# smhassanerfani/nasa-niswan

Hardware: AMD Instinct MI355X
Metric: training samples/sec (90x144x20 grid, seq_len=12) (higher is better)
Workload: dtype bf16; 1 GPU; cfg1-20level; in_channels=62, out_channels=20, seq_len=12, batch_per_gpu=8, global_batch=8, parallelism=dp1, wave=4, overlap_allreduce=False

## Files before the change

nasa-niswan_amd/csrc/conv_igemm.hip:

```cpp
#include "nint_common.h"

enum { EPI_LSTM = 0, EPI_DGRAD = 1, EPI_DGRAD_PW = 2 };

#ifndef NINT_TINY_AUTO
#define NINT_TINY_AUTO(dtype) ((dtype) == NINT_F32)
#endif
#ifndef NINT_STENCIL_AUTO
#define NINT_STENCIL_AUTO(dtype) false
#endif

#ifndef NINT_BD
#define NINT_BD 3
#endif
constexpr int BD_WIDE = NINT_BD;
constexpr int BD_NARROW = 2;
#ifndef NINT_AG
#define NINT_AG 2
#endif
#ifndef NINT_ABUF
#define NINT_ABUF 2
#endif

#ifdef NINT_STAMP
#define NINT_STAMP_WGS 4096
// ... 11 lines not shown
extern "C" int nint_debug_read_hwid(unsigned* host, int n_wgs) {
  if (!host || n_wgs <= 0 || n_wgs > NINT_STAMP_WGS) return NINT_E_ARG;
  NINT_CHECK_HIP(hipDeviceSynchronize());
  NINT_CHECK_HIP(hipMemcpyFromSymbol(host, HIP_SYMBOL(g_hwid), (size_t)n_wgs * 2 * sizeof(unsigned)));
  return NINT_OK;
}
extern "C" int nint_debug_read_stamps(unsigned long long* host, int n_wgs) {
  if (!host || n_wgs <= 0 || n_wgs > NINT_STAMP_WGS) return NINT_E_ARG;
  NINT_CHECK_HIP(hipDeviceSynchronize());
  NINT_CHECK_HIP(hipMemcpyFromSymbol(host, HIP_SYMBOL(g_stamp), (size_t)n_wgs * 8 * sizeof(unsigned long long)));
  return NINT_OK;
}
#else
#define NINT_STAMP_AT(slot)
#endif

template <int DT> struct Pk4;
template <> struct Pk4<NINT_F32> {
  typedef f32x4_t T;
  static __device__ __forceinline__ T ld(const void* p, size_t i) { return *(const f32x4_t*)((const float*)p + i); }
  static __device__ __forceinline__ f32x4_t up(T v) { return v; }
  static __device__ __forceinline__ T zero() { return (f32x4_t){0.f, 0.f, 0.f, 0.f}; }
};
template <> struct Pk4<NINT_BF16> {
  typedef u32x2_t T;
  static __device__ __forceinline__ T ld(const void* p, size_t i) { return *(const u32x2_t*)((const uint16_t*)p + i); }
  static __device__ __forceinline__ f32x4_t up(T w) {
    return (f32x4_t){__builtin_bit_cast(float, w[0] << 16), __builtin_bit_cast(float, w[0] & 0xffff0000u),
                     __builtin_bit_cast(float, w[1] << 16), __builtin_bit_cast(float, w[1] & 0xffff0000u)};
  }
  static __device__ __forceinline__ T zero() { return (u32x2_t){0u, 0u}; }
};

constexpr int xchg_rounds(int EPI, int WK, int NTW, int MT) {
  return (WK == 4 && MT == 4 && NTW % 2 == 0) ? 2 : ((WK == 4 && MT == 8 && NTW == 4) ? 4 : 1);
}

template <int DT, int EPI, int WN, int WK, int NTW, int MT>
__device__ __forceinline__ void conv_igemm_body(const ConvArgs& a, char* smem, const int bx_, const int by_, const int nbx_) {
  static_assert(WN * WK == 4, "four waves per workgroup");
  constexpr int BD = MT >= 8 ? BD_WIDE : BD_NARROW;
  static_assert(EPI != EPI_LSTM || NTW % 4 == 0, "LSTM epilogue needs the 4 gate tiles in one wave");
  constexpr int NTH = 256;
  constexpr int NTWG = WN * NTW;
  constexpr int Q = MT / WK;
  static_assert(MT % WK == 0, "K-slice waves split the tile rows evenly");

  const int tid = threadIdx.x, lane = tid & 63;
  NINT_STAMP_AT(0)
  const int wave = __builtin_amdgcn_readfirstlane(tid >> 6);
  const int wn = wave % WN, wk = wave / WN;
  int tile;
  {
    const int nb = nbx_, b = bx_, q8 = nb / 8, r8 = nb % 8, x = b % 8, i = b / 8;
    tile = x * q8 + (x < r8 ? x : r8) + i;
  }
  const bool mg = MT >= 8 && tile >= a.n_full;
  int tx, ty, img;
  if (!mg) {
    tx = tile % a.tiles_x; tile /= a.tiles_x;
    ty = tile % a.tiles_full_y;
    img = tile / a.tiles_full_y;
  } else {
    tile -= a.n_full;
    tx = tile % a.tiles_x2;
    img = tile / a.tiles_x2;
    ty = a.tiles_full_y;
  }
  constexpr int RHM = MT >= 8 ? MT / 2 : MT;
  const int nt0 = a.nt_begin + by_ * NTWG + wn * NTW;
  const int y0 = ty * MT, x0 = mg ? tx * 32 : tx * 16;
  auto rdy = [&](int r) __attribute__((always_inline)) { return mg ? r % RHM : r; };
// ... 60 lines not shown
        const int r = (i + wk * Q) % MT;
        const int y = y0 + rdy(r), x = x0 + rdx(r) + (lane & 15);
        const size_t rowpix = ((size_t)img * a.H + y) * a.W;
#pragma unroll
        for (int j = 0; j < NTW; ++j) {
          const int n = (nt0 + j) * 16 + c4;
          old[i][j] = (f32x4_t){0.f, 0.f, 0.f, 0.f};
          if (rmw && n < a.C0p && y < a.H && x < a.W)
            old[i][j] = load_vec4<DT>(a.out0 + rowpix * a.C0p * Elem<DT>::ES, (unsigned)(x * a.C0p + n));
        }
      }
    }
  };
  if constexpr (EARLY) load_cprev();
  for (int c_begin = 0; c_begin < nchunks; c_begin += a.cpf) {
    const int c_cnt = min(a.cpf, nchunks - c_begin);
    if (c_begin > 0) __syncthreads();
    const int a_units = c_cnt * 4 * NHPp;
    for (int ub = wave * 64; ub < a_units; ub += 4 * 64) {
      const int u = ub + lane;
      const int cq = (int)__umulhi((unsigned)u, magic_nhpp);
      int hp = u - cq * NHPp;
      hp = hp < NHP ? hp : 0;
      const int q = cq & 3, cl = cq >> 2;
      const int hy = (int)__umulhi((unsigned)hp, magic_hwt);
      const int hx = hp - hy * HWt;
      const int c = c_begin + cl;
      const char* src = (c < a.nchunk0)
          ? base0 + ((long)hy * a.Wh + hx) * a.pix_stride0 + c * 64 + q * 16
          : base1 + ((long)hy * a.Wh + hx) * a.pix_stride1 + (c - a.nchunk0) * 64 + q * 16;
      __builtin_amdgcn_global_load_lds((const __attribute__((address_space(1))) void*)src,
                                       (__attribute__((address_space(3))) void*)(smem + (size_t)ub * 16), 16, 0, 0);
    }
    const int n0f = a.kx0 == k ? 0 : min(max(a.nchunk0 - c_begin, 0), c_cnt);
    const int steps_before = min(c_begin, a.nchunk0) * k * a.kx0 + max(c_begin - a.nchunk0, 0) * taps;
    bool synced = false;
    for (int seg = 0; seg < 2; ++seg) {
    const int cs_lo = seg == 0 ? 0 : n0f, cs_n = seg == 0 ? n0f : c_cnt - n0f;
    if (cs_n == 0) continue;
    const int kx = seg == 0 ? a.kx0 : k;
    const int xoff = kx == k ? 0 : p;
    const int tps = k * kx;
    const int nsteps = cs_n * tps;
    const int s_lo = (nsteps * wk) / WK, s_hi = (nsteps * (wk + 1)) / WK;
    int cl = s_lo / tps;
    int tap = s_lo - cl * tps;
    cl += cs_lo;
    int tyy = tap / kx;
    int txx = tap - tyy * kx;
    const char* Bs = Bwave + (size_t)(steps_before + (seg == 0 ? 0 : n0f * k * a.kx0) + s_lo) * bstep;
    u32x4_t bq[BD][NTW];
    int b_rem = s_hi - 1 - s_lo;
    const char* Bn = Bs;
#define NINT_B_ADVANCE() { const bool adv_ = b_rem > 0; b_rem -= adv_ ? 1 : 0; Bn += adv_ ? bstep : 0; }
    if (s_lo < s_hi) {
#pragma unroll
      for (int d = 0; d < BD; ++d) {
#pragma unroll
        for (int j = 0; j < NTW; ++j) bq[d][j] = *(const u32x4_t*)(Bn + blane + j * 1024);
        NINT_B_ADVANCE()
      }
    }
    if (!synced) {
      __syncthreads();
      synced = true;
      if (c_begin == 0) { NINT_STAMP_AT(1) }
// ... 90 lines not shown
    }
    }
  }

#undef NINT_B_ADVANCE
  NINT_STAMP_AT(2)
  if constexpr (WK > 1) {
    constexpr int FR = MT - Q;
    constexpr int XR = xchg_rounds(EPI, WK, NTW, MT), NTX = NTW / XR;
    __syncthreads();
#pragma unroll
    for (int xr = 0; xr < XR; ++xr) {
      if (xr > 0) __syncthreads();
      char* mine = smem + (size_t)((wn * WK + wk) * FR * NTX) * 1024 + lane * 16;
#pragma unroll
      for (int ii = Q; ii < MT; ++ii)
#pragma unroll
        for (int j = 0; j < NTX; ++j) *(f32x4_t*)(mine + ((ii - Q) * NTX + j) * 1024) = acc[ii][xr * NTX + j];
      __syncthreads();
#pragma unroll
      for (int d = 1; d < WK; ++d) {
        const int src = (wk + d) % WK;
        const int shift = ((wk - src + WK) % WK) * Q;
        const char* theirs = smem + (size_t)((wn * WK + src) * FR * NTX) * 1024 + lane * 16;
#pragma unroll
        for (int ii = 0; ii < Q; ++ii)
#pragma unroll
          for (int j = 0; j < NTX; ++j)
            acc[ii][xr * NTX + j] += *(const f32x4_t*)(theirs + ((ii + shift - Q) * NTX + j) * 1024);
      }
    }
  }

  if constexpr (!EARLY) load_cprev();
  load_old();
  const int px = lane & 15;
  const int c4 = 4 * (lane >> 4);
  const int x = x0 + px;
  if constexpr (EPI == EPI_LSTM) {
#pragma unroll
    for (int cb = 0; cb < NTW / 4; ++cb) {
      const int cblock = nt0 / 4 + cb;
      const int ch = cblock * 16 + c4;
      const int Gc = 4 * a.Ch16;
      const int odd = (lane >> 4) & 1, chb = (lane >> 5) * 8;
      const unsigned lo_c = (unsigned)(x * a.Chp + ch);
      const unsigned lo_h = (unsigned)((x + a.P) * a.Chp + ch);
      const unsigned lo_g = (unsigned)(x * Gc + cblock * 64) + (DT == NINT_BF16 ? (unsigned)(chb + (odd ? 32 : 0)) : (unsigned)c4);
#pragma unroll
      for (int i = 0; i < Q; ++i) {
        const int rt = (i + wk * Q) % MT;
        const int y = y0 + rdy(rt), xo = rdx(rt);
        const bool ok = y < a.H && x + xo < a.W;
        const size_t rowpix = ((size_t)img * a.H + y) * a.W + xo;
        const f32x4_t cp = cpv[i][cb];
        f32x4_t gi, gf, gg, go, cn, hn;
#pragma unroll
        for (int r = 0; r < 4; ++r) {
          gi[r] = sigmoidf_(acc[i][cb * 4 + 0][r]);
          gf[r] = sigmoidf_(acc[i][cb * 4 + 1][r]);
          gg[r] = tanhf_(acc[i][cb * 4 + 2][r]);
          go[r] = sigmoidf_(acc[i][cb * 4 + 3][r]);
          cn[r] = fmaf(cp[r], gf[r], gi[r] * gg[r]);
          hn[r] = go[r] * tanhf_(cn[r]);
        }
        if (ok) {
// ... 168 lines not shown
  int i = 0;                                                                                                    \
  _Pragma("unroll") for (int q = 1; q < NINT_MULTI_MAX; ++q) i += (q < m.n && (int)blockIdx.x >= m.begin[q]) ? 1 : 0; \
  const int b = blockIdx.x - m.begin[i];                                                                        \
  if (b >= m.nwg[i]) return;                                        \
  const int nbx = m.nbx[i], by = b / nbx, bx = b - by * nbx;                                                    \
  const ConvArgs& a = m.a[i];
#define NINT_MULTI_CASE(EPI_, WN_, WK_, NTW_) \
  case conv_variant(EPI_, WN_, WK_, NTW_, 4): conv_igemm_body<DT, EPI_, WN_, WK_, NTW_, 4>(a, smem, bx, by, nbx); break;
template <int DT>
__global__ __launch_bounds__(256, 3) void conv_lstm_multi_kernel(ConvMulti m) {
  NINT_MULTI_PROLOGUE
  switch (m.variant[i]) {
    NINT_MULTI_CASE(EPI_LSTM, 4, 1, 4)
    NINT_MULTI_CASE(EPI_LSTM, 2, 2, 4)
    NINT_MULTI_CASE(EPI_LSTM, 1, 4, 4)
    default: break;
  }
}
#define NINT_MULTI_CASE8(EPI_, WN_, WK_, NTW_) \
  case conv_variant(EPI_, WN_, WK_, NTW_, 8): conv_igemm_body<DT, EPI_, WN_, WK_, NTW_, 8>(a, smem, bx, by, nbx); break;
template <int DT>
__global__ __launch_bounds__(256, 2) void conv_lstm_multi8_kernel(ConvMulti m) {
  NINT_MULTI_PROLOGUE
  switch (m.variant[i]) {
    NINT_MULTI_CASE8(EPI_LSTM, 4, 1, 4)
    NINT_MULTI_CASE8(EPI_LSTM, 2, 2, 4)
    NINT_MULTI_CASE8(EPI_LSTM, 1, 4, 4)
    NINT_MULTI_CASE(EPI_LSTM, 4, 1, 4)
    NINT_MULTI_CASE(EPI_LSTM, 2, 2, 4)
    NINT_MULTI_CASE(EPI_LSTM, 1, 4, 4)
    default: break;
  }
}
template <int DT>
__global__ __launch_bounds__(256, 3) void conv_bwd_multi_kernel(ConvMulti m) {
  if (m.pw_blocks && (int)blockIdx.x >= m.begin[m.n]) {
#ifndef NINT_PW_U
#define NINT_PW_U 2
#endif
    lstm_bwd_pointwise_body<DT, NINT_PW_U>(m.pw, blockIdx.x - m.begin[m.n], m.pw_blocks);
    return;
  }
  NINT_MULTI_PROLOGUE
  switch (m.variant[i]) {
    NINT_MULTI_CASE(EPI_DGRAD, 1, 4, 4)
    NINT_MULTI_CASE(EPI_DGRAD, 1, 4, 2)
    NINT_MULTI_CASE(EPI_DGRAD, 2, 2, 3)
    NINT_MULTI_CASE(EPI_DGRAD, 1, 4, 3)
    NINT_MULTI_CASE(EPI_DGRAD_PW, 1, 4, 3)
    default: break;
  }
}
template <int DT>
__global__ __launch_bounds__(256, 2) void conv_bwd_multi8_kernel(ConvMulti m) {
  NINT_MULTI_PROLOGUE
  switch (m.variant[i]) {
    NINT_MULTI_CASE8(EPI_DGRAD, 1, 4, 4)
    NINT_MULTI_CASE8(EPI_DGRAD_PW, 1, 4, 3)
    NINT_MULTI_CASE(EPI_DGRAD, 1, 4, 4)
    NINT_MULTI_CASE(EPI_DGRAD, 1, 4, 2)
    NINT_MULTI_CASE(EPI_DGRAD_PW, 1, 4, 3)
    default: break;
  }
}
template <int DT>
__global__ __launch_bounds__(256, 2) void conv_dgrad_multi8_kernel(ConvMulti m) {
  NINT_MULTI_PROLOGUE
  switch (m.variant[i]) {
    NINT_MULTI_CASE8(EPI_DGRAD, 1, 4, 4)
    NINT_MULTI_CASE8(EPI_DGRAD, 2, 2, 3)
    default: break;
  }
}
static bool multi_holds(int variant) {
  switch (variant) {
    case conv_variant(EPI_LSTM, 4, 1, 4, 8): case conv_variant(EPI_DGRAD, 1, 4, 4, 8):
    case conv_variant(EPI_LSTM, 2, 2, 4, 8): case conv_variant(EPI_LSTM, 1, 4, 4, 8): case conv_variant(EPI_DGRAD_PW, 1, 4, 3, 8):
    case conv_variant(EPI_LSTM, 4, 1, 4, 4): case conv_variant(EPI_LSTM, 2, 2, 4, 4): case conv_variant(EPI_LSTM, 1, 4, 4, 4):
    case conv_variant(EPI_DGRAD, 1, 4, 4, 4): case conv_variant(EPI_DGRAD, 1, 4, 2, 4): case conv_variant(EPI_DGRAD_PW, 1, 4, 3, 4):
    case conv_variant(EPI_DGRAD, 2, 2, 3, 8): case conv_variant(EPI_DGRAD, 2, 2, 3, 4):
    case conv_variant(EPI_DGRAD, 1, 4, 3, 4):
      return true;
// ... 120 lines not shown
  a.k = ly->k; a.p = ly->k / 2; a.taps = ly->k * ly->k;
  a.kx0 = ly->xfold ? 1 : ly->k;
  a.H = g->H; a.W = g->W; a.P = g->P; a.Hh = g->Hh; a.Wh = g->Wh;
  a.bias = ly->bias_p;
  a.c_prev = c_prev; a.c_out = c_out; a.h_out = (char*)h_out; a.gates_out = (char*)gates_out;
  a.Chp = ly->Chp; a.Ch16 = ly->Ch16;
  a.tile_rows = ly->tile_rows <= 2 ? 0 : ly->tile_rows;
  if (ly->wide < 0 || ly->wide > 2) return NINT_E_ARG;
  if (nint_internal_stencil_holds(ly) && (ly->tile_rows == 1 || (ly->tile_rows == 0 && NINT_STENCIL_AUTO(dtype)))) {
    if (plan) { plan->gx = 0; plan->carrier = NINT_K_STENCIL; return NINT_E_SHAPE; }
    return nint_internal_stencil_lstm(ly, g, dtype, N, x_slab, h_prev, c_prev, h_out, c_out, gates_out, stream);
  }
  if ((ly->tile_rows == 2 || (ly->tile_rows == 0 && NINT_TINY_AUTO(dtype))) && nint_tiny_shape(ly->Cx, ly->Ch, ly->k, ly->xfold, dtype)) {
    if (plan) { plan->gx = 0; plan->carrier = NINT_K_TINY; return NINT_E_SHAPE; }
    return nint_internal_tiny_lstm(ly, g, dtype, N, x_slab, h_prev, c_prev, h_out, c_out, gates_out, stream);
  }
  ConvPlan own;
  ConvPlan* pl = plan ? plan : &own;
  const int rc = dtype == NINT_BF16 ? launch_conv<NINT_BF16, EPI_LSTM>(a, N, a.NTt, n_cu, pl)
                                    : launch_conv<NINT_F32, EPI_LSTM>(a, N, a.NTt, n_cu, pl);
  return rc != NINT_OK || plan ? rc : nint_internal_conv_enqueue(pl, stream);
}

extern "C" int nint_cell_fwd(const nint_layer* ly, const nint_geom* g, int dtype, int N,
                             const void* x_slab, const void* h_prev, const float* c_prev,
                             void* h_out, float* c_out, void* gates_out, void* stream) {
  return cell_fwd(ly, g, dtype, N, x_slab, h_prev, c_prev, h_out, c_out, gates_out, stream, 0, nullptr);
}

int nint_internal_cell_fwd_plan(const CellFwdJob* j, const nint_geom* g, int dtype, int N, int n_cu, ConvPlan* plan) {
  return cell_fwd(j->ly, g, dtype, N, j->x_slab, j->h_prev, j->c_prev, j->h_out, j->c_out, j->gates_out, nullptr, n_cu, plan);
}

int nint_internal_multi_plan(const ConvPlan* plans, int n, const PwArgs* pw, MultiPlan* out) {
  if (!plans || n < 1 || n > NINT_MULTI_MAX) return NINT_E_SHAPE;
  ConvMulti& m = out->m;
  m = ConvMulti{};
  size_t lds = 0;
  int b = 0, nfwd = 0;
  for (int i = 0; i < n; ++i) {
    const ConvPlan& pl = plans[i];
    if (pl.gx <= 0 || !multi_holds(pl.variant)) return NINT_E_SHAPE;
    nfwd += pl.variant / 10000 == EPI_LSTM ? 1 : 0;
    m.a[i] = pl.a; m.variant[i] = pl.variant; m.nbx[i] = pl.gx; m.nwg[i] = pl.gx * pl.gy;
    m.begin[i] = b;
    b += nint_round_up(pl.gx * pl.gy, 8);
    if (pl.lds > lds) lds = pl.lds;
  }
  if (nfwd != 0 && nfwd != n) return NINT_E_SHAPE;
  if (pw && nfwd) return NINT_E_SHAPE;
  m.n = n;
  for (int i = n; i <= NINT_MULTI_MAX; ++i) m.begin[i] = b;
  bool rows8 = false, dpair = false;
  for (int i = 0; i < n; ++i) rows8 = rows8 || plans[i].variant % 10 == 2;
  for (int i = 0; i < n; ++i) dpair = dpair || plans[i].variant == conv_variant(EPI_DGRAD, 2, 2, 3, 8);
  for (int i = 0; i < n; ++i)
    if (rows8 && (plans[i].variant == conv_variant(EPI_DGRAD, 2, 2, 3, 4) || plans[i].variant == conv_variant(EPI_DGRAD, 1, 4, 3, 4))) return NINT_E_SHAPE;
  if (dpair)
    for (int i = 0; i < n; ++i)
      if (plans[i].variant != conv_variant(EPI_DGRAD, 2, 2, 3, 8) && plans[i].variant != conv_variant(EPI_DGRAD, 1, 4, 4, 8)) return NINT_E_SHAPE;
  if (pw) {
    if (rows8 || dpair) return NINT_E_SHAPE;
    const size_t total = (size_t)pw->N * pw->H * pw->W * (pw->Ch16 / 4);
    size_t pb = (total + 255) / 256;
    const size_t want = (size_t)b;
    if (pb > want) pb = want < (pb + 3) / 4 ? (pb + 3) / 4 : want;
    m.pw = *pw; m.pw_blocks = (int)pb;
    b += (int)pb;
  }
  out->grid = b; out->lds = lds;
  out->carrier = dpair ? NINT_K_CONV_DGRAD_MULTI8
                       : nfwd ? (rows8 ? NINT_K_CONV_LSTM_MULTI8 : NINT_K_CONV_LSTM_MULTI) : (rows8 ? NINT_K_CONV_BWD_MULTI8 : NINT_K_CONV_BWD_MULTI);
  return NINT_OK;
}

template <int DT>
static const void* multi_kernel(int carrier) {
  switch (carrier) {
    case NINT_K_CONV_DGRAD_MULTI8: return (const void*)conv_dgrad_multi8_kernel<DT>;
    case NINT_K_CONV_LSTM_MULTI8: return (const void*)conv_lstm_multi8_kernel<DT>;
    case NINT_K_CONV_LSTM_MULTI: return (const void*)conv_lstm_multi_kernel<DT>;
    case NINT_K_CONV_BWD_MULTI8: return (const void*)conv_bwd_multi8_kernel<DT>;
    default: return (const void*)conv_bwd_multi_kernel<DT>;
  }
}
int nint_internal_multi_enqueue(const MultiPlan* mp, int dtype, void* stream) {
  const void* kern = dtype == NINT_BF16 ? multi_kernel<NINT_BF16>(mp->carrier) : multi_kernel<NINT_F32>(mp->carrier);
  if (mp->lds > 64 * 1024) NINT_CHECK_HIP(hipFuncSetAttribute(kern, hipFuncAttributeMaxDynamicSharedMemorySize, (int)mp->lds));
  void* args[] = {(void*)&mp->m};
  (void)hipLaunchKernel(kern, dim3(mp->grid), dim3(256), args, mp->lds, (hipStream_t)stream);
  NINT_LAUNCH_CHECK();
  return NINT_OK;
}

static int dgrad_now(const nint_layer* ly, const nint_geom* g, int dtype, int N, const void* dG, void* dx_accum, void* dh_prev,
                     bool overwrite_dx, const DgradPw* pw, void* stream) {
  ConvPlan pl;
// ... 65 lines not shown
```

nasa-niswan_amd/csrc/nint_common.h:

```cpp
#pragma once
#include <hip/hip_runtime.h>
#include <stdint.h>
#include <type_traits>
#include "nint.h"

typedef __attribute__((ext_vector_type(8))) __bf16 bf16x8_t;
typedef __attribute__((ext_vector_type(4))) float f32x4_t;
typedef __attribute__((ext_vector_type(4))) uint32_t u32x4_t;
typedef __attribute__((ext_vector_type(2))) uint32_t u32x2_t;
typedef __attribute__((ext_vector_type(4))) short s16x4_t;

#define NINT_CHECK_HIP(expr)                      \
  do {                                            \
    hipError_t _e = (expr);                       \
    if (_e != hipSuccess) return (int)_e;         \
  } while (0)

#define NINT_LAUNCH_CHECK()                       \
  do {                                            \
    hipError_t _e = hipGetLastError();            \
    if (_e != hipSuccess) return (int)_e;         \
  } while (0)

template <int DT> struct Elem;
// ... 53 lines not shown
  w[1] = pack_bf16x2(v[2], v[3]);
  *(u32x2_t*)((uint16_t*)p + i) = w;
}

template <int DT> __device__ __forceinline__ f32x4_t load_vec4(const void* p, size_t i);
template <> __device__ __forceinline__ f32x4_t load_vec4<NINT_F32>(const void* p, size_t i) { return *(const f32x4_t*)((const float*)p + i); }
template <> __device__ __forceinline__ f32x4_t load_vec4<NINT_BF16>(const void* p, size_t i) {
  const u32x2_t w = *(const u32x2_t*)((const uint16_t*)p + i);
  return (f32x4_t){__builtin_bit_cast(float, w[0] << 16), __builtin_bit_cast(float, w[0] & 0xffff0000u),
                   __builtin_bit_cast(float, w[1] << 16), __builtin_bit_cast(float, w[1] & 0xffff0000u)};
}

template <int DT> __device__ __forceinline__ f32x4_t mma_step(u32x4_t a, u32x4_t b, f32x4_t c);
template <> __device__ __forceinline__ f32x4_t mma_step<NINT_BF16>(u32x4_t a, u32x4_t b, f32x4_t c) {
  return __builtin_amdgcn_mfma_f32_16x16x32_bf16(__builtin_bit_cast(bf16x8_t, a), __builtin_bit_cast(bf16x8_t, b), c, 0, 0, 0);
}
template <> __device__ __forceinline__ f32x4_t mma_step<NINT_F32>(u32x4_t a, u32x4_t b, f32x4_t c) {
  f32x4_t af = __builtin_bit_cast(f32x4_t, a), bf = __builtin_bit_cast(f32x4_t, b);
  c = __builtin_amdgcn_mfma_f32_16x16x4f32(af[0], bf[0], c, 0, 0, 0);
  c = __builtin_amdgcn_mfma_f32_16x16x4f32(af[1], bf[1], c, 0, 0, 0);
  c = __builtin_amdgcn_mfma_f32_16x16x4f32(af[2], bf[2], c, 0, 0, 0);
  c = __builtin_amdgcn_mfma_f32_16x16x4f32(af[3], bf[3], c, 0, 0, 0);
  return c;
}

__device__ __forceinline__ float rcpf_(float x) { return __builtin_amdgcn_rcpf(x); }
__device__ __forceinline__ float sigmoidf_(float x) { return rcpf_(1.0f + __expf(-x)); }
__device__ __forceinline__ float tanhf_(float x) { return fmaf(2.0f, rcpf_(1.0f + __expf(-2.0f * x)), -1.0f); }

struct PwArgs {
  const void* gates; const float* c_prev; const float* c_new; const void* dh; const void* dh2; float* dc; void* dG;
  int N, H, W, P, Hh, Wh, Ch16, Chp, dc_zero;
};
template <int DT, int U = 1>
__device__ __forceinline__ void lstm_bwd_pointwise_body(const PwArgs& a, size_t blk, size_t nblk) {
  const int nq = a.Ch16 >> 2;
  const size_t total = (size_t)a.N * a.H * a.W * nq;
  const int Gc = 4 * a.Ch16;
  const size_t stride = nblk * 256;
  for (size_t i0 = blk * 256 + threadIdx.x; i0 < total; i0 += stride * U) {
    f32x4_t gi[U], gf[U], gg[U], go[U], cp[U], cn[U], dhv[U], dcv[U];
    size_t ci[U], ob[U];
    bool on[U];
#pragma unroll
    for (int u = 0; u < U; ++u) {
      const size_t i = i0 + (size_t)u * stride;
      on[u] = i < total;
      if (!on[u]) continue;
      const int q = i % nq;
      const size_t pix = i / nq;
      const int x = pix % a.W;
      size_t r = pix / a.W;
      const int y = r % a.H;
      const int n = r / a.H;
      const int ch = 4 * q;
      const int cblock = ch >> 4, col = ch & 15;
      const size_t gb = pix * Gc + (size_t)cblock * 64 + col;
      gi[u] = load_vec4<DT>(a.gates, gb);
      gf[u] = load_vec4<DT>(a.gates, gb + 16);
      gg[u] = load_vec4<DT>(a.gates, gb + 32);
      go[u] = load_vec4<DT>(a.gates, gb + 48);
      ci[u] = pix * a.Chp + ch;
      cp[u] = (f32x4_t){0.f, 0.f, 0.f, 0.f};
      if (a.c_prev) cp[u] = *(const f32x4_t*)(a.c_prev + ci[u]);
      cn[u] = *(const f32x4_t*)(a.c_new + ci[u]);
      dhv[u] = load_vec4<DT>(a.dh, ci[u]);
      if (a.dh2) dhv[u] += load_vec4<DT>(a.dh2, ci[u]);
      dcv[u] = (f32x4_t){0.f, 0.f, 0.f, 0.f};
      if (!a.dc_zero) dcv[u] = *(const f32x4_t*)(a.dc + ci[u]);
      ob[u] = ((((size_t)n * a.Hh) + (y + a.P)) * a.Wh + (x + a.P)) * Gc + (size_t)cblock * 64 + col;
    }
#pragma unroll
    for (int u = 0; u < U; ++u) {
      if (!on[u]) continue;
      f32x4_t o_i, o_f, o_g, o_o, dcp;
#pragma unroll
      for (int e = 0; e < 4; ++e) {
        const float tc = tanhf_(cn[u][e]);
        const float dct = dcv[u][e] + dhv[u][e] * go[u][e] * (1.f - tc * tc);
        const float d_o = dhv[u][e] * tc;
        o_i[e] = dct * gg[u][e] * gi[u][e] * (1.f - gi[u][e]);
        o_f[e] = dct * cp[u][e] * gf[u][e] * (1.f - gf[u][e]);
        o_g[e] = dct * gi[u][e] * (1.f - gg[u][e] * gg[u][e]);
        o_o[e] = d_o * go[u][e] * (1.f - go[u][e]);
        dcp[e] = dct * gf[u][e];
      }
      store_vec4<DT>(a.dG, ob[u], o_i);
      store_vec4<DT>(a.dG, ob[u] + 16, o_f);
      store_vec4<DT>(a.dG, ob[u] + 32, o_g);
      store_vec4<DT>(a.dG, ob[u] + 48, o_o);
      *(f32x4_t*)(a.dc + ci[u]) = dcp;
    }
  }
}

struct ConvArgs {
  const char* src0;
  const char* src1;
  int nchunk0, nchunk1;
  long img_stride0, img_stride1;
  int pix_stride0, pix_stride1;
  const char* Bp;
  int NTt;
  int nt_begin;
// ... 67 lines not shown
__host__ __device__ inline size_t nint_tiny_bytes() { return (size_t)NINT_TINY_MAXSTEPS * 2 * 1024 + 4 * NINT_TINY_MAXSTEPS * sizeof(int) + 64; }
__host__ __device__ inline size_t nint_internal_tiny_offset(int Cx, int Cxp, int Ch, int Chp, int Ch16, int k, int xfold, int dtype) {
  const size_t o = nint_internal_stencil_offset(Cxp, Chp, Ch16, k, dtype) + ((size_t)3 * nint_stencil_rows(Cx, Ch, xfold) + 1) * 128;
  return (o + 255) / 256 * 256;
}
int nint_internal_tiny_lstm(const nint_layer* ly, const nint_geom* g, int dtype, int N, const void* x_slab,
                            const void* h_prev, const float* c_prev, void* h_out, float* c_out, void* gates_out,
                            void* stream);
bool nint_internal_stencil_holds(const nint_layer* ly);
int nint_internal_stencil_lstm(const nint_layer* ly, const nint_geom* g, int dtype, int N, const void* x_slab,
                               const void* h_prev, const float* c_prev, void* h_out, float* c_out, void* gates_out,
                               void* stream);
#define NINT_MULTI_MAX 4
struct CellFwdJob {
  const nint_layer* ly; const void* x_slab; const void* h_prev; const float* c_prev; void* h_out; float* c_out; void* gates_out;
};
struct ConvPlan {
  ConvArgs a; int gx, gy; size_t lds; int variant;
  const void* kern;
  int carrier;
};
constexpr int conv_variant(int EPI, int WN, int WK, int NTW, int MT) { return EPI * 10000 + WN * 1000 + WK * 100 + NTW * 10 + MT / 4; }
int nint_internal_n_cu();
int nint_internal_cell_fwd_plan(const CellFwdJob* j, const nint_geom* g, int dtype, int N, int n_cu, ConvPlan* plan);
int nint_internal_conv_enqueue(const ConvPlan* plan, void* stream);
struct ConvMulti {
  ConvArgs a[NINT_MULTI_MAX];
  int n;
  int begin[NINT_MULTI_MAX + 1];
  int nbx[NINT_MULTI_MAX];
  int nwg[NINT_MULTI_MAX];
  int variant[NINT_MULTI_MAX];
  PwArgs pw;
  int pw_blocks;
};
struct MultiPlan { ConvMulti m; int carrier, grid; size_t lds; };
int nint_internal_multi_plan(const ConvPlan* plans, int n, const PwArgs* pw, MultiPlan* out);
int nint_internal_multi_enqueue(const MultiPlan* mp, int dtype, void* stream);
struct DgradPw {
  const void* gates; const float* c_prev; const float* c_new; float* dc; const void* old; void* dG_out;
  const void* lo_gates; const float* lo_c_prev; const float* lo_c_new; float* lo_dc; void* lo_dG_out; int lo_Ch16; bool lo_dc_zero;
  int tile_rows;
};
int nint_internal_conv_dgrad(const nint_layer* ly, const nint_geom* g, int dtype, int N, const void* dG, void* dx_accum,
                             void* dh_prev, bool overwrite_dx, const DgradPw* pw, int n_cu, ConvPlan* plan);
```

nasa-niswan_amd/csrc/seq.hip:

```cpp
#include <string.h>
#include <vector>
#include "nint_common.h"

extern "C" int nint_version(void) { return NINT_VERSION; }

extern "C" const char* nint_error_string(int code) {
  switch (code) {
    case NINT_OK: return "ok";
    case NINT_E_ARG: return "nint: invalid argument";
    case NINT_E_SHAPE: return "nint: shape not supported by any kernel instantiation";
    case NINT_E_LDS: return "nint: tile does not fit in LDS";
    case NINT_E_ALIGN: return "nint: pointer not 16-byte aligned";
    default: return code > 0 ? hipGetErrorString((hipError_t)code) : "nint: unknown error";
  }
}

extern "C" int nint_device_info(int* n_cu, int* lds_bytes_per_cu, int* wave_size, char* name, int name_len) {
  int dev = 0;
  NINT_CHECK_HIP(hipGetDevice(&dev));
  hipDeviceProp_t prop;
  NINT_CHECK_HIP(hipGetDeviceProperties(&prop, dev));
  if (n_cu) *n_cu = prop.multiProcessorCount;
  if (lds_bytes_per_cu) *lds_bytes_per_cu = (int)prop.maxSharedMemoryPerMultiProcessor;
  if (wave_size) *wave_size = prop.warpSize;
// ... 81 lines not shown
  if (!s->xs) return NINT_E_ARG;
  for (int l = 0; l < s->L; ++l) {
    if (!s->h[l] || !s->c[l]) return NINT_E_ARG;
    if (l > 0 && s->layer[l].Cxp != s->layer[l - 1].Chp) return NINT_E_ARG;
  }
  return NINT_OK;
}

enum { STEP_CONV, STEP_MULTI, STEP_PW, STEP_GATE };
struct SeqProb { int op, layer, t; };
struct GateCall { CellFwdJob job; nint_layer ly; int carrier; };
struct SeqStep {
  int kind;
  int probe, tag_layer, tag_t;
  int n; SeqProb prob[NINT_MULTI_MAX + 1];
  union { ConvPlan conv; MultiPlan multi; PwArgs pw; GateCall gate; };
};
typedef std::vector<SeqStep> Steps;

static SeqStep& push(Steps& out, int kind, int probe, int tag_layer, int tag_t) {
  SeqStep& st = out.emplace_back();
  st.kind = kind; st.probe = probe; st.tag_layer = tag_layer; st.tag_t = tag_t;
  return st;
}
static void push_conv(Steps& out, const ConvPlan& pl, int probe, int op, int l, int t) {
  if (pl.gx <= 0) return;
  SeqStep& st = push(out, STEP_CONV, probe, l, t);
  st.prob[st.n++] = SeqProb{op, l, t}; st.conv = pl;
}
static void push_pw(Steps& out, const PwArgs& pa, int l, int t) {
  SeqStep& st = push(out, STEP_PW, NINT_PROBE_POINTWISE, l, t);
  st.prob[st.n++] = SeqProb{NINT_OP_POINTWISE, l, t}; st.pw = pa;
}
static bool push_grid(Steps& out, const ConvPlan* plans, int n, const PwArgs* pw, int probe, int tag_layer, int tag_t, const SeqProb* prob, int np) {
  SeqStep& st = push(out, STEP_MULTI, probe, tag_layer, tag_t);
  if (nint_internal_multi_plan(plans, n, pw, &st.multi) != NINT_OK) { out.pop_back(); return false; }
  for (; st.n < np; ++st.n) st.prob[st.n] = prob[st.n];
  return true;
}

static int run_steps(const nint_seq* s, const Steps& steps, Probe& probe, void* stream) {
  for (const SeqStep& st : steps) {
    probe.stamp(st.probe, st.tag_layer, st.tag_t, 0);
    int rc = NINT_E_ARG;
    switch (st.kind) {
      case STEP_CONV: rc = nint_internal_conv_enqueue(&st.conv, stream); break;
      case STEP_MULTI: rc = nint_internal_multi_enqueue(&st.multi, s->dtype, stream); break;
      case STEP_PW: rc = nint_internal_pointwise_enqueue(&st.pw, s->dtype, stream); break;
      case STEP_GATE: rc = nint_cell_fwd(&st.gate.ly, &s->g, s->dtype, s->B, st.gate.job.x_slab, st.gate.job.h_prev, st.gate.job.c_prev,
                                         st.gate.job.h_out, st.gate.job.c_out, st.gate.job.gates_out, stream); break;
    }
    probe.stamp(st.probe, st.tag_layer, st.tag_t, 1);
    if (rc != NINT_OK) return rc;
  }
  return NINT_OK;
}

static int plan_gate(const nint_seq* s, int n_cu, bool rows8, int l, int t, GateCall* gc, ConvPlan* pl) {
  const nint_geom* g = &s->g;
  const size_t es = esize(s->dtype), halo_px = (size_t)g->Hh * g->Wh, comp_px = (size_t)g->H * g->W, B = s->B;
  gc->ly = s->layer[l];
  const nint_layer* ly = &gc->ly;
  if (rows8 && ly->tile_rows == 0) gc->ly.tile_rows = 8;
  const size_t hs = (size_t)B * halo_px * ly->Chp * es, cs = (size_t)B * comp_px * ly->Chp;
  const bool zero_state = (t == 0 && !s->has_init_state);
  CellFwdJob& j = gc->job; j.ly = ly;
  j.x_slab = (l == 0) ? (const char*)s->xs + (size_t)t * B * halo_px * ly->Cxp * es
                      : (const char*)s->h[l - 1] + (size_t)(t + 1) * B * halo_px * ly->Cxp * es;
  j.h_prev = zero_state ? nullptr : (const char*)s->h[l] + (size_t)t * hs; j.c_prev = zero_state ? nullptr : s->c[l] + (size_t)t * cs;
// ... 5 lines not shown
}

static int plan_fwd(const nint_seq* s, int n_cu, Steps& out) {
  const int L = s->L, T = s->T;
  const bool wavefront = s->wave && L > 1 && L <= NINT_MULTI_MAX;
  const bool rows8 = wavefront && (s->wave == 2 || s->wave == 3 || s->wave == 4);
  out.reserve((size_t)T * L);
  for (int w = 0; w < (wavefront ? T + L - 1 : T * L); ++w) {
    GateCall gc[NINT_MULTI_MAX]; ConvPlan pl[NINT_MULTI_MAX]; SeqProb pr[NINT_MULTI_MAX];
    int n = 0; bool planned = true;
    for (int l = wavefront ? 0 : w % L; l < (wavefront ? L : w % L + 1); ++l) {
      const int t = wavefront ? w - l : w / L;
      if (t < 0 || t >= T) continue;
      const int rc = plan_gate(s, n_cu, rows8, l, t, &gc[n], &pl[n]);
      if (rc != NINT_OK && rc != NINT_E_SHAPE) return rc;
      planned = planned && rc == NINT_OK;
      pr[n++] = SeqProb{NINT_OP_GATE, l, t};
    }
    if (n > 1 && planned && push_grid(out, pl, n, nullptr, NINT_PROBE_WAVE, n, w, pr, n)) continue;
    for (int q = 0; q < n; ++q) {
      if (pl[q].gx > 0) { push_conv(out, pl[q], NINT_PROBE_GATE, NINT_OP_GATE, pr[q].layer, pr[q].t); continue; }
      SeqStep& st = push(out, STEP_GATE, NINT_PROBE_GATE, pr[q].layer, pr[q].t);
      st.prob[st.n++] = pr[q]; st.gate = gc[q]; st.gate.job.ly = nullptr;
    }
  }
  return NINT_OK;
}


#ifndef NINT_AUTO_LO
#define NINT_AUTO_LO true
#endif

static int bwd_check(const nint_seq* s) {
  const int rc = seq_check(s);
  if (rc != NINT_OK) return rc;
  for (int l = 0; l < s->L; ++l)
    if (!s->gates[l] || !s->dG[l] || !s->dh[l] || !s->dc[l] || !s->dW[l] || !s->db[l]) return NINT_E_ARG;
  if ((s->need_dx && !s->dx) || !s->wg_partial) return NINT_E_ARG;
  if (s->fuse_bwd < 0 || (s->fuse_bwd > 2 && !(s->fuse_bwd & 0x40000000)) || s->bwd_parts < 0 || s->bwd_parts > 2) return NINT_E_ARG;
  if ((((uintptr_t)s->dh_seq) & 15) != 0) return NINT_E_ALIGN;
  return NINT_OK;
}

struct BwdPlanner {
  const nint_seq* s; int n_cu; Steps& out;
  int L, T; size_t B, es, halo_px, comp_px;
  bool fused[NINT_MAX_LAYERS];
  bool lo[NINT_MAX_LAYERS], loc[NINT_MAX_LAYERS];
  int off[NINT_MAX_LAYERS], pw_done[NINT_MAX_LAYERS];
  bool merge, merge_d, merge_p;
  void* dh0_own;
  bool has_d, has_p;
  ConvPlan held_d; int held_u;
  PwArgs held_p; int held_t;

  BwdPlanner(const nint_seq* s_, int n_cu_, Steps& out_) : s(s_), n_cu(n_cu_), out(out_), L(s_->L), T(s_->T), B(s_->B), has_d(false), has_p(false), held_u(0), held_t(0) {
    es = esize(s->dtype); halo_px = (size_t)s->g.Hh * s->g.Wh; comp_px = (size_t)s->g.H * s->g.W;
    const bool explicit_mask = (s->fuse_bwd & 0x40000000) != 0;
    for (int l = L - 1; l >= 0; --l) {
      const nint_layer* ly = &s->layer[l];
      const int ksteps = (4 * ly->Ch16 / (s->dtype == NINT_BF16 ? 32 : 16)) * ly->k * ly->k;
      fused[l] = explicit_mask ? ((s->fuse_bwd >> l) & 1) != 0 : (s->fuse_bwd == 2 || (s->fuse_bwd == 0 && ksteps <= 24));
      off[l] = (l == L - 1 ? 0 : off[l + 1]) + (fused[l] ? 1 : 0);
      pw_done[l] = -1;
    }
    for (int l = 0; l < L; ++l) {
      lo[l] = fused[l] && l > 0 && !fused[l - 1] && (explicit_mask ? ((s->fuse_bwd >> (8 + l)) & 1) != 0 : NINT_AUTO_LO);
      loc[l] = !fused[l] && l > 0 && !fused[l - 1] && explicit_mask && ((s->fuse_bwd >> (16 + l)) & 1) != 0;
    }
    merge = (s->wave == 1 || s->wave == 3) && L >= 3 && fused[L - 1] && !fused[0] && !loc[0];
    const size_t dh0_bytes = (size_t)B * comp_px * s->layer[0].Chp * es;
    merge_d = (s->wave == 4 || s->wave == 5) && L >= 2 && !fused[0] && !fused[1] && !loc[0] && !loc[1] && s->wg_partial_bytes >= dh0_bytes;
    merge_p = merge_d && L >= 3 && fused[L - 1];
    dh0_own = merge_d ? (void*)s->wg_partial : s->dh[0];
  }

  void flush_d() { if (has_d) push_conv(out, held_d, NINT_PROBE_DGRAD, NINT_OP_DGRAD, 0, held_u); has_d = false; }
  void flush_p() { if (has_p) push_pw(out, held_p, 0, held_t); has_p = false; }

  const void* seq_block(int l, int t) const {
    return s->dh_seq && l == L - 1 ? (const char*)s->dh_seq + (size_t)t * B * comp_px * s->layer[l].Chp * es : nullptr;
  }

  int pointwise(int l, int t, int so) {
    if (!merge_d || l == 0) flush_d();
    const nint_layer* ly = &s->layer[l];
    const size_t cs = (size_t)B * comp_px * ly->Chp, Gc = 4 * (size_t)ly->Ch16;
    PwArgs pa;
    const void* blk = seq_block(l, t);
    const void* dh = blk && t == T - 1 ? blk : s->dh[l];
    const void* dh2 = merge_d && l == 0 && t < T - 1 ? dh0_own : (blk && t < T - 1 ? blk : nullptr);
    const int rc = nint_internal_pointwise_plan(ly, &s->g, s->dtype, B, (const char*)s->gates[l] + (size_t)t * B * comp_px * Gc * es,
                                                s->c[l] + (size_t)t * cs, s->c[l] + (size_t)(t + 1) * cs, dh, s->dc[l],
                                                (char*)s->dG[l] + (size_t)t * B * halo_px * Gc * es, t == T - 1 && ((s->zero_dstate >> (2 * l)) & 1),
                                                dh2, &pa);
    if (rc != NINT_OK) return rc;
    if (merge_p && l == 0 && so + off[L - 1] >= 2) { has_p = true; held_p = pa; held_t = t; }
    else push_pw(out, pa, l, t);
    return NINT_OK;
  }

  void ride_lo(DgradPw& pw, int l, int u) {
    const nint_layer* lb = &s->layer[l - 1];
    const size_t cs_b = (size_t)B * comp_px * lb->Chp, Gc_b = 4 * (size_t)lb->Ch16;
    pw.lo_gates = (const char*)s->gates[l - 1] + (size_t)u * B * comp_px * Gc_b * es;
    pw.lo_c_prev = s->c[l - 1] + (size_t)u * cs_b; pw.lo_c_new = s->c[l - 1] + (size_t)(u + 1) * cs_b;
// ... 21 lines not shown
  }

  int classic(int l, int u, int so) {
    int rc = pw_done[l] != u ? pointwise(l, u, so) : (int)NINT_OK;
    if (rc != NINT_OK) return rc;
    DgradPw pw = {};
    if (loc[l]) { ride_lo(pw, l, u); pw.tile_rows = 4; }
    ConvPlan pl;
    rc = dgrad(l, u, loc[l] ? &pw : nullptr, &pl);
    if (rc != NINT_OK) return rc;
    if (merge_d && l == 1 && has_d && pair(pl, NINT_OP_DGRAD, l, u)) return NINT_OK;
    if (!merge_d || l <= 1) flush_d();
    if ((merge || merge_d) && l == 0 && so > -off[0]) { has_d = pl.gx > 0; held_d = pl; held_u = u; }
    else push_conv(out, pl, NINT_PROBE_DGRAD, NINT_OP_DGRAD, l, u);
    return NINT_OK;
  }

  int fused_step(int l, int u) {
    const nint_layer* ly = &s->layer[l];
    const size_t cs = (size_t)B * comp_px * ly->Chp, Gc = 4 * (size_t)ly->Ch16;
    DgradPw pw = {};
    pw.gates = (const char*)s->gates[l] + (size_t)(u - 1) * B * comp_px * Gc * es; pw.c_prev = s->c[l] + (size_t)(u - 1) * cs;
    pw.c_new = s->c[l] + (size_t)u * cs; pw.dc = s->dc[l]; pw.old = l < L - 1 ? s->dh[l] : seq_block(l, u - 1);
    pw.dG_out = (char*)s->dG[l] + (size_t)(u - 1) * B * halo_px * Gc * es;
    if (lo[l]) ride_lo(pw, l, u);
    const bool top_pair = merge && has_d && l == L - 1;
    if (top_pair && s->wave == 3) pw.tile_rows = 8;
    ConvPlan pl;
    const int rc = dgrad(l, u, &pw, &pl);
    if (rc != NINT_OK) return rc;
    if (top_pair && pair(pl, NINT_OP_FUSED, l, u)) return NINT_OK;
    if (!merge_d) flush_d();
    const SeqProb pr[2] = {{NINT_OP_FUSED, l, u}, {NINT_OP_POINTWISE, 0, held_t}};
    if (has_p && push_grid(out, &pl, 1, &held_p, NINT_PROBE_BWD_PW, l, u, pr, 2)) { has_p = false; return NINT_OK; }
    flush_p();
    push_conv(out, pl, NINT_PROBE_FUSED, NINT_OP_FUSED, l, u);
    return NINT_OK;
  }

  int plan() {
    out.reserve((size_t)(T + L) * L * 2);
    for (int so = T - 1; so >= -off[0] && s->bwd_parts != 2; --so) {
      for (int l = L - 1; l >= 0; --l) {
        const int u = so + off[l];
        if (u < 0 || u > (fused[l] ? T : T - 1)) continue;
        if (!(l == L - 1 && u >= 1 && u < T)) flush_p();
        int rc = NINT_OK;
        if (!fused[l]) rc = classic(l, u, so);
        else if (u == T) rc = pointwise(l, T - 1, so);
        else if (u >= 1) rc = fused_step(l, u);
        else {
          if (!merge_d) flush_d();
          ConvPlan pl;
          if ((rc = dgrad(l, 0, nullptr, &pl)) == NINT_OK) push_conv(out, pl, NINT_PROBE_DGRAD, NINT_OP_DGRAD, l, 0);
        }
        if (rc != NINT_OK) return rc;
      }
    }
    flush_p(); flush_d();
    return NINT_OK;
  }
};

static int plan_pass(const nint_seq* s, bool bwd, Steps& steps) {
  const int rc = bwd ? bwd_check(s) : seq_check(s);
  if (rc != NINT_OK) return rc;
  const int n_cu = nint_internal_n_cu();
// ... 59 lines not shown
```

Measured before the change: 1055 samples/s.

## Let conv dgrad workgroups ride a slice of the backward LSTM pointwise work

Adds a rider hook in the implicit-GEMM conv body so the fused dgrad+pointwise conv workgroups process a capped chunk of the pending LSTM backward pointwise kernel while their LDS loads are in flight. The remaining pointwise elements stay on dedicated tail blocks. The goal is to hide the pointwise memory traffic behind conv load latency and shrink the extra block count. It also raises the bf16 occupancy hint on the backward multi kernel, which constrains registers. The riding is gated behind a flag that defaults off.

```diff
diff --git a/nasa-niswan_amd/csrc/conv_igemm.hip b/nasa-niswan_amd/csrc/conv_igemm.hip
--- a/nasa-niswan_amd/csrc/conv_igemm.hip
+++ b/nasa-niswan_amd/csrc/conv_igemm.hip
@@ -67,12 +67,30 @@
   static __device__ __forceinline__ T zero() { return (u32x2_t){0u, 0u}; }
 };
 
+#ifndef NINT_PW_U
+#define NINT_PW_U 2
+#endif
+#ifndef NINT_PW_RIDE_U
+#define NINT_PW_RIDE_U 1
+#endif
+#ifndef NINT_PW_RIDE_CAP
+#define NINT_PW_RIDE_CAP 4
+#endif
+#ifndef NINT_PW_RIDE_SPLIT
+#define NINT_PW_RIDE_SPLIT 0
+#endif
+#ifndef NINT_BWD_MULTI_WGS
+#define NINT_BWD_MULTI_WGS(DT) ((DT) == NINT_BF16 ? 4 : 3)
+#endif
+
 constexpr int xchg_rounds(int EPI, int WK, int NTW, int MT) {
   return (WK == 4 && MT == 4 && NTW % 2 == 0) ? 2 : ((WK == 4 && MT == 8 && NTW == 4) ? 4 : 1);
 }
 
-template <int DT, int EPI, int WN, int WK, int NTW, int MT>
-__device__ __forceinline__ void conv_igemm_body(const ConvArgs& a, char* smem, const int bx_, const int by_, const int nbx_) {
+struct NoRider { __device__ __forceinline__ void operator()(int) const {} };
+template <int DT, int EPI, int WN, int WK, int NTW, int MT, class RIDER = NoRider>
+__device__ __forceinline__ void conv_igemm_body(const ConvArgs& a, char* smem, const int bx_, const int by_, const int nbx_,
+                                                const RIDER& rider = RIDER()) {
   static_assert(WN * WK == 4, "four waves per workgroup");
   constexpr int BD = MT >= 8 ? BD_WIDE : BD_NARROW;
   static_assert(EPI != EPI_LSTM || NTW % 4 == 0, "LSTM epilogue needs the 4 gate tiles in one wave");
@@ -199,6 +217,7 @@
       __builtin_amdgcn_global_load_lds((const __attribute__((address_space(1))) void*)src,
                                        (__attribute__((address_space(3))) void*)(smem + (size_t)ub * 16), 16, 0, 0);
     }
+    if (c_begin == 0) rider(0);
     const int n0f = a.kx0 == k ? 0 : min(max(a.nchunk0 - c_begin, 0), c_cnt);
     const int steps_before = min(c_begin, a.nchunk0) * k * a.kx0 + max(c_begin - a.nchunk0, 0) * taps;
     bool synced = false;
@@ -355,6 +374,9 @@
     }
   }
 
+#if NINT_PW_RIDE_SPLIT
+  rider(1);
+#endif
   if constexpr (!EARLY) load_cprev();
   load_old();
   const int px = lane & 15;
@@ -589,13 +611,30 @@
     default: break;
   }
 }
+template <int DT> struct PwRider {
+  const ConvMulti& m;
+  __device__ __forceinline__ void operator()(int phase) const {
+    if (!m.pw_ride_end) return;
+#if NINT_PW_RIDE_SPLIT
+    const size_t mid = (size_t)m.begin[1] * 256 * NINT_PW_RIDE_SPLIT;
+    if (phase == 0) lstm_bwd_pointwise_body<DT, NINT_PW_RIDE_U, true>(m.pw, blockIdx.x, m.begin[1], 0, mid < m.pw_ride_end ? mid : m.pw_ride_end);
+    else if (mid < m.pw_ride_end) lstm_bwd_pointwise_body<DT, NINT_PW_RIDE_U, true>(m.pw, blockIdx.x, m.begin[1], mid, m.pw_ride_end);
+#else
+    lstm_bwd_pointwise_body<DT, NINT_PW_RIDE_U, true>(m.pw, blockIdx.x, m.begin[1], 0, m.pw_ride_end);
+#endif
+  }
+};
 template <int DT>
-__global__ __launch_bounds__(256, 3) void conv_bwd_multi_kernel(ConvMulti m) {
+__global__ __launch_bounds__(256, NINT_BWD_MULTI_WGS(DT)) void conv_bwd_multi_kernel(ConvMulti m) {
   if (m.pw_blocks && (int)blockIdx.x >= m.begin[m.n]) {
-#ifndef NINT_PW_U
-#define NINT_PW_U 2
-#endif
-    lstm_bwd_pointwise_body<DT, NINT_PW_U>(m.pw, blockIdx.x - m.begin[m.n], m.pw_blocks);
+    lstm_bwd_pointwise_body<DT, NINT_PW_U>(m.pw, blockIdx.x - m.begin[m.n], m.pw_blocks, m.pw_ride_end);
+    return;
+  }
+  if (m.pw_ride_end && (int)blockIdx.x >= m.nwg[0]) {
+    PwRider<DT>{m}(0);
+#if NINT_PW_RIDE_SPLIT
+    PwRider<DT>{m}(1);
+#endif
     return;
   }
   NINT_MULTI_PROLOGUE
@@ -604,7 +643,7 @@
     NINT_MULTI_CASE(EPI_DGRAD, 1, 4, 2)
     NINT_MULTI_CASE(EPI_DGRAD, 2, 2, 3)
     NINT_MULTI_CASE(EPI_DGRAD, 1, 4, 3)
-    NINT_MULTI_CASE(EPI_DGRAD_PW, 1, 4, 3)
+    case conv_variant(EPI_DGRAD_PW, 1, 4, 3, 4): conv_igemm_body<DT, EPI_DGRAD_PW, 1, 4, 3, 4>(a, smem, bx, by, nbx, PwRider<DT>{m}); break;
     default: break;
   }
 }
@@ -791,7 +830,7 @@
   return cell_fwd(j->ly, g, dtype, N, j->x_slab, j->h_prev, j->c_prev, j->h_out, j->c_out, j->gates_out, nullptr, n_cu, plan);
 }
 
-int nint_internal_multi_plan(const ConvPlan* plans, int n, const PwArgs* pw, MultiPlan* out) {
+int nint_internal_multi_plan(const ConvPlan* plans, int n, const PwArgs* pw, bool pw_ride, MultiPlan* out) {
   if (!plans || n < 1 || n > NINT_MULTI_MAX) return NINT_E_SHAPE;
   ConvMulti& m = out->m;
   m = ConvMulti{};
@@ -821,7 +860,13 @@
   if (pw) {
     if (rows8 || dpair) return NINT_E_SHAPE;
     const size_t total = (size_t)pw->N * pw->H * pw->W * (pw->Ch16 / 4);
-    size_t pb = (total + 255) / 256;
+    size_t rest = total;
+    if (pw_ride && n == 1 && plans[0].variant == conv_variant(EPI_DGRAD_PW, 1, 4, 3, 4)) {
+      const size_t cap = (size_t)b * 256 * NINT_PW_RIDE_CAP;
+      m.pw_ride_end = total < cap ? total : cap;
+      rest = total - m.pw_ride_end;
+    }
+    size_t pb = (rest + 255) / 256;
     const size_t want = (size_t)b;
     if (pb > want) pb = want < (pb + 3) / 4 ? (pb + 3) / 4 : want;
     m.pw = *pw; m.pw_blocks = (int)pb;
diff --git a/nasa-niswan_amd/csrc/nint_common.h b/nasa-niswan_amd/csrc/nint_common.h
--- a/nasa-niswan_amd/csrc/nint_common.h
+++ b/nasa-niswan_amd/csrc/nint_common.h
@@ -109,13 +109,13 @@
   const void* gates; const float* c_prev; const float* c_new; const void* dh; const void* dh2; float* dc; void* dG;
   int N, H, W, P, Hh, Wh, Ch16, Chp, dc_zero;
 };
-template <int DT, int U = 1>
-__device__ __forceinline__ void lstm_bwd_pointwise_body(const PwArgs& a, size_t blk, size_t nblk) {
+template <int DT, int U = 1, bool DRAIN = false>
+__device__ __forceinline__ void lstm_bwd_pointwise_body(const PwArgs& a, size_t blk, size_t nblk, size_t first = 0, size_t end = 0) {
   const int nq = a.Ch16 >> 2;
-  const size_t total = (size_t)a.N * a.H * a.W * nq;
+  const size_t total = end ? end : (size_t)a.N * a.H * a.W * nq;
   const int Gc = 4 * a.Ch16;
   const size_t stride = nblk * 256;
-  for (size_t i0 = blk * 256 + threadIdx.x; i0 < total; i0 += stride * U) {
+  for (size_t i0 = first + blk * 256 + threadIdx.x; i0 < total; i0 += stride * U) {
     f32x4_t gi[U], gf[U], gg[U], go[U], cp[U], cn[U], dhv[U], dcv[U];
     size_t ci[U], ob[U];
     bool on[U];
@@ -147,6 +147,7 @@
       if (!a.dc_zero) dcv[u] = *(const f32x4_t*)(a.dc + ci[u]);
       ob[u] = ((((size_t)n * a.Hh) + (y + a.P)) * a.Wh + (x + a.P)) * Gc + (size_t)cblock * 64 + col;
     }
+    if constexpr (DRAIN) asm volatile("s_waitcnt vmcnt(0)" ::: "memory");
 #pragma unroll
     for (int u = 0; u < U; ++u) {
       if (!on[u]) continue;
@@ -280,10 +281,11 @@
   int nwg[NINT_MULTI_MAX];
   int variant[NINT_MULTI_MAX];
   PwArgs pw;
+  size_t pw_ride_end;
   int pw_blocks;
 };
 struct MultiPlan { ConvMulti m; int carrier, grid; size_t lds; };
-int nint_internal_multi_plan(const ConvPlan* plans, int n, const PwArgs* pw, MultiPlan* out);
+int nint_internal_multi_plan(const ConvPlan* plans, int n, const PwArgs* pw, bool pw_ride, MultiPlan* out);
 int nint_internal_multi_enqueue(const MultiPlan* mp, int dtype, void* stream);
 struct DgradPw {
   const void* gates; const float* c_prev; const float* c_new; float* dc; const void* old; void* dG_out;
diff --git a/nasa-niswan_amd/csrc/seq.hip b/nasa-niswan_amd/csrc/seq.hip
--- a/nasa-niswan_amd/csrc/seq.hip
+++ b/nasa-niswan_amd/csrc/seq.hip
@@ -137,9 +137,10 @@
   SeqStep& st = push(out, STEP_PW, NINT_PROBE_POINTWISE, l, t);
   st.prob[st.n++] = SeqProb{NINT_OP_POINTWISE, l, t}; st.pw = pa;
 }
-static bool push_grid(Steps& out, const ConvPlan* plans, int n, const PwArgs* pw, int probe, int tag_layer, int tag_t, const SeqProb* prob, int np) {
+static bool push_grid(Steps& out, const ConvPlan* plans, int n, const PwArgs* pw, int probe, int tag_layer, int tag_t, const SeqProb* prob, int np,
+                      bool pw_ride = true) {
   SeqStep& st = push(out, STEP_MULTI, probe, tag_layer, tag_t);
-  if (nint_internal_multi_plan(plans, n, pw, &st.multi) != NINT_OK) { out.pop_back(); return false; }
+  if (nint_internal_multi_plan(plans, n, pw, pw_ride, &st.multi) != NINT_OK) { out.pop_back(); return false; }
   for (; st.n < np; ++st.n) st.prob[st.n] = prob[st.n];
   return true;
 }
@@ -211,6 +212,10 @@
 #define NINT_AUTO_LO true
 #endif
 
+#ifndef NINT_AUTO_PW_RIDE
+#define NINT_AUTO_PW_RIDE false
+#endif
+
 static int bwd_check(const nint_seq* s) {
   const int rc = seq_check(s);
   if (rc != NINT_OK) return rc;
@@ -228,7 +233,7 @@
   bool fused[NINT_MAX_LAYERS];
   bool lo[NINT_MAX_LAYERS], loc[NINT_MAX_LAYERS];
   int off[NINT_MAX_LAYERS], pw_done[NINT_MAX_LAYERS];
-  bool merge, merge_d, merge_p;
+  bool merge, merge_d, merge_p, pw_blocks;
   void* dh0_own;
   bool has_d, has_p;
   ConvPlan held_d; int held_u;
@@ -252,6 +257,7 @@
     const size_t dh0_bytes = (size_t)B * comp_px * s->layer[0].Chp * es;
     merge_d = (s->wave == 4 || s->wave == 5) && L >= 2 && !fused[0] && !fused[1] && !loc[0] && !loc[1] && s->wg_partial_bytes >= dh0_bytes;
     merge_p = merge_d && L >= 3 && fused[L - 1];
+    pw_blocks = explicit_mask ? ((s->fuse_bwd >> 24) & 1) != 0 : !NINT_AUTO_PW_RIDE;
     dh0_own = merge_d ? (void*)s->wg_partial : s->dh[0];
   }
 
@@ -339,7 +345,7 @@
     if (top_pair && pair(pl, NINT_OP_FUSED, l, u)) return NINT_OK;
     if (!merge_d) flush_d();
     const SeqProb pr[2] = {{NINT_OP_FUSED, l, u}, {NINT_OP_POINTWISE, 0, held_t}};
-    if (has_p && push_grid(out, &pl, 1, &held_p, NINT_PROBE_BWD_PW, l, u, pr, 2)) { has_p = false; return NINT_OK; }
+    if (has_p && push_grid(out, &pl, 1, &held_p, NINT_PROBE_BWD_PW, l, u, pr, 2, !pw_blocks)) { has_p = false; return NINT_OK; }
     flush_p();
     push_conv(out, pl, NINT_PROBE_FUSED, NINT_OP_FUSED, l, u);
     return NINT_OK;
```

New measurement: 1032 samples/s. 2.2% lower.
